# pramasoul/lac

Hardware: AMD Instinct MI355X
Metric: encoded symbols/sec at vocab=32000, batch=4096 streams; bit-exact round-trip (higher is better)
Workload: dtype u32; 1 GPU; c3: vocab=32000, 4096 streams/GPU, 16 symbols/stream per job, prec=48, uint32 pmf rows; vocab=32000, streams=4096, prec=48, pmf_bits=32, input=pmf, parallelism=streams sharded over 1 GPU(s)

## Files before the change

### lac_amd/csrc/lac_encode.hip

```cpp
#include "lac_host.h"
#include "lac_drain.h"
#include "lac_wire.h"

#include <type_traits>

namespace {

#if LAC_ENC_PHASES
__device__ unsigned long long g_enc_phase[8];
#endif

template <typename E, int VEC>
__global__ __launch_bounds__(256) void k_row_stats(const E *__restrict__ pmf, int64_t step_stride,
                                                   int64_t stream_stride, const int32_t *__restrict__ sym,
                                                   int64_t B, int64_t rows, int64_t V, int64_t t0,
                                                   RowStats *__restrict__ out, const EncState *states,
                                                   const int64_t *__restrict__ slen) {
    const int lane = (int)lane_id();
    const int64_t r = (int64_t)blockIdx.x * kWavesPerBlock + (threadIdx.x >> 6);
    if (r >= rows) return;
    const int64_t t = t0 + r / B, b = r % B;
    if (slen && !live_row(slen, b, states[b].nsym, r / B)) return;
    const RowSums rs = row_reduce<E, VEC>(pmf + t * step_stride + b * stream_stride, V, sym[t * B + b]);
    if (lane == 0) {
        RowStats st;
        if (rs.T >> 64) {
            st.lo = st.hi = st.tot = 0;
            st.minp = 1;
        } else {
            st.lo = (uint64_t)rs.lo;
            st.hi = (uint64_t)rs.lo + rs.ps;
            st.tot = (uint64_t)rs.T;
            st.minp = rs.T ? rs.minp : 0;
        }
        st.inv_tot = st.tot ? 1.0 / (double)st.tot : 0.0;
        st.pad = 0;
        out[r] = st;
    }
}

struct SP {
    uint64_t lo, hi, tot, flo, fhi, fthr;
    int n, prec;
    uint64_t cap_words, *pa, *pc;
    int lane;
};
template <bool CEIL, bool T32, bool FT>
__device__ inline int straight_steps(const SP &sp, EncState &st, int64_t &l, int64_t &h, bool &ok) {
    auto store = [&](uint64_t idx, uint64_t wa, uint64_t wc) {
        if (sp.lane == 0) { sp.pa[idx] = wa; sp.pc[idx] = wc; }
    };
    typedef typename std::conditional<T32, uint32_t, uint64_t>::type CT;
    struct Row {
        CT lo, hi, T;
        uint64_t fl, fh, ft;
    };
    auto rd = [&](int j) {
        Row r;
        if constexpr (T32) {
            r.lo = (uint32_t)__builtin_amdgcn_readlane((int)(uint32_t)sp.lo, j);
            r.hi = (uint32_t)__builtin_amdgcn_readlane((int)(uint32_t)sp.hi, j);
            r.T = (uint32_t)__builtin_amdgcn_readlane((int)(uint32_t)sp.tot, j);
        } else {
            r.lo = readlane_u64(sp.lo, j);
            r.hi = readlane_u64(sp.hi, j);
            r.T = readlane_u64(sp.tot, j);
        }
        r.fl = readlane_u64(sp.flo, j);
        r.fh = readlane_u64(sp.fhi, j);
        r.ft = FT ? readlane_u64(sp.fthr, j) : 0;
        return r;
    };
    const int n = sp.n, prec = sp.prec;
    const int64_t nsym0 = st.nsym;
    Row nx = rd(0);
    int i = 0;
    int kk = 0;
    uint64_t e = 0;
    bool fudged = false;
    while (i < n) {
        for (; i < n; i++) {
            const Row r = nx;
            nx = rd(i + 1 < n ? i + 1 : i);
            const uint64_t w = (uint64_t)(h - l + 1);
            if constexpr (FT) {
                if (!nonneg_uni((int64_t)(w - r.ft))) {
                    fudged = true;
                    break;
                }
            }
            uint64_t a, bb;
            if constexpr (T32) {
                a = frac_mul_div32<CEIL>(r.fl, r.lo, w, r.T);
                bb = frac_mul_div32<CEIL>(r.fh, r.hi, w, r.T);
            } else {
                a = frac_mul_div<true>(r.fl, r.lo, w, r.T, CEIL);
                bb = frac_mul_div<true>(r.fh, r.hi, w, r.T, CEIL);
            }
            h = l + (int64_t)bb - 1;
            l = l + (int64_t)a;
            const uint64_t d = (uint64_t)(h - l);
            const int sh = bitlen64(d);
            kk = prec - sh;
            e = kk > 0 ? (uint64_t)l >> sh : 0;
            l = (int64_t)(((uint64_t)l - (e << sh)) << kk);
            h = l + (int64_t)((d + 1) << kk) - 1;
            const int off0 = (int)(st.L & 63);
            const int avail = off0 ? 64 - off0 : 0;
            if (__builtin_expect(kk > avail, 0)) break;
            st.wc |= (e >> kk) << ((64 - off0) & 63);
            st.wa |= (e & ((1ull << kk) - 1)) << ((64 - off0 - kk) & 63);
            st.L += (uint64_t)kk;
        }
        if (i >= n) break;
        if constexpr (FT) {
            if (fudged) break;
        }
        if (!plane_append(st.L, st.wa, st.wc, kk, e, sp.cap_words, store)) {
            st.err = LAC_E_CAPACITY;
            ok = false;
            break;
        }
        i++;
    }
    st.nsym = nsym0 + i;
    return i;
}

template <typename E, int MAP>
__global__ __launch_bounds__(256) void k_encode(const RowStats *__restrict__ stats, const int32_t *__restrict__ sym,
                                                int64_t B, int64_t t0, int64_t nsteps, const E *pmf,
                                                int64_t step_stride, int64_t stream_stride, int64_t V, int prec,
                                                EncState *states, uint64_t *planeA, uint64_t *planeC,
                                                uint64_t cap_words, uint64_t *trace, int mapping,
                                                bool allow_fudge, const int64_t *__restrict__ slen) {
    const int lane = (int)lane_id();
    const int64_t b = (int64_t)blockIdx.x * kWavesPerBlock + wave_in_block();
    if (b >= B) return;
    EncState st = states[b];
    if (slen) {
        nsteps = live_steps(slen, b, st.nsym, nsteps);
        if (nsteps == 0) return;
    }
    if (st.err || st.nflush >= 0) {
        if (lane == 0 && !st.err && st.nflush >= 0) { st.err = LAC_E_STATE; st.err_step = st.nsym; states[b] = st; }
        return;
    }
    uint64_t *pa = planeA + (uint64_t)b * cap_words, *pc = planeC + (uint64_t)b * cap_words;
    int64_t l = (int64_t)rfl_u64((uint64_t)st.l), h = (int64_t)rfl_u64((uint64_t)st.h);
    st.L = rfl_u64(st.L);
    st.wa = rfl_u64(st.wa);
    st.wc = rfl_u64(st.wc);
    st.nsym = (int64_t)rfl_u64((uint64_t)st.nsym);
#if LAC_ENC_PHASES
    PhaseClock clock, *clk = &clock;
    clock.start();
#else
    NoClock *clk = nullptr;
#endif
    bool ok = true;
    for (int64_t g0 = 0; g0 < nsteps && ok; g0 += 64) {
        const int n = (int)((nsteps - g0) < 64 ? (nsteps - g0) : 64);
        RowStats my = {0, 0, 0, 0, 0.0, 0};
        int32_t mys = 0;
        if (lane < n) {
            my = stats[(g0 + lane) * B + b];
            mys = sym[(t0 + g0 + lane) * B + b];
        }
        const bool frac_ok = lane < n && !(my.tot >> 62);
        const uint64_t flo = frac_ok ? row_frac(my.lo, my.tot) : kNoFrac;
        const uint64_t fhi = frac_ok ? row_frac(my.hi, my.tot) : kNoFrac;
        int i0 = 0;
        if constexpr (sizeof(E) == 8) {
            const uint64_t half = 1ull << (prec - 1);
            const bool lfast = lane >= n || (frac_ok && my.tot != 0 && my.hi > my.lo && (uint32_t)mys < (uint32_t)V &&
                                             (MAP != LAC_MAP_FLOOR || ((my.tot - 1) >> (prec - 1)) < my.hi - my.lo));
            const uint64_t d0 = (uint64_t)(h - l);
            if (!trace && prec <= 61 && __ballot(!lfast) == 0 && nonneg_uni((int64_t)(d0 - half)) &&
                !(d0 >> prec)) {
                constexpr bool CEIL = MAP != LAC_MAP_FLOOR;
                const bool t32 = __ballot(lane < n && (my.tot >> 32)) == 0;
                const bool ft = CEIL && __ballot(lane < n && my.tot > half) != 0;
                uint64_t ftl = 0;
                if (ft) {
                    ftl = lane < n && my.minp ? div_floor((u128)my.tot + (my.minp - 1), my.minp) : 0;
                    ftl = ftl < (1ull << 62) ? ftl : (1ull << 62);
                }
                SP sp{my.lo, my.hi, my.tot, flo, fhi, ftl, n, prec, cap_words, pa, pc, lane};
                if (t32)
                    i0 = ft ? straight_steps<CEIL, true, true>(sp, st, l, h, ok)
                            : straight_steps<CEIL, true, false>(sp, st, l, h, ok);
                else
                    i0 = ft ? straight_steps<CEIL, false, true>(sp, st, l, h, ok)
                            : straight_steps<CEIL, false, false>(sp, st, l, h, ok);
                if (!ok || i0 >= n) continue;
            }
        }
        if (i0 == 0) {
            const uint64_t half = 1ull << (prec - 1);
            const bool lfast = lane >= n || (frac_ok && my.tot != 0 && my.tot <= half && !(my.tot >> 32) &&
                                             my.hi > my.lo && (uint32_t)mys < (uint32_t)V);
            const uint64_t d0 = (uint64_t)(h - l);
            if (!trace && prec <= 61 && __ballot(!lfast) == 0 && nonneg_uni((int64_t)(d0 - half)) &&
                !(d0 >> prec)) {
                constexpr bool CEIL = MAP != LAC_MAP_FLOOR;
                const int64_t nsym0 = st.nsym;
                auto store = [&](uint64_t idx, uint64_t wa, uint64_t wc) {
                    if (lane == 0) { pa[idx] = wa; pc[idx] = wc; }
                };
                auto rd = [&](int j, uint32_t &lo, uint32_t &hi, uint32_t &T, uint64_t &fl, uint64_t &fh) {
                    lo = (uint32_t)__builtin_amdgcn_readlane((int)(uint32_t)my.lo, j);
                    hi = (uint32_t)__builtin_amdgcn_readlane((int)(uint32_t)my.hi, j);
                    T = (uint32_t)__builtin_amdgcn_readlane((int)(uint32_t)my.tot, j);
                    fl = readlane_u64(flo, j);
                    fh = readlane_u64(fhi, j);
                };
                uint32_t nlo, nhi, nT;
                uint64_t nfl, nfh;
                rd(0, nlo, nhi, nT, nfl, nfh);
                int i = 0;
                int kk = 0;
                uint64_t e = 0;
                while (i < n) {
                    for (; i < n; i++) {
                        uint32_t lo, hi, T;
                        uint64_t fl, fh;
                        lo = nlo, hi = nhi, T = nT, fl = nfl, fh = nfh;
                        rd(i + 1 < n ? i + 1 : i, nlo, nhi, nT, nfl, nfh);
                        const uint64_t w = (uint64_t)(h - l + 1);
                        const uint64_t a = frac_mul_div32<CEIL>(fl, lo, w, T), bb = frac_mul_div32<CEIL>(fh, hi, w, T);
                        h = l + (int64_t)bb - 1;
                        l = l + (int64_t)a;
                        const uint64_t d = (uint64_t)(h - l);
                        const int sh = bitlen64(d);
                        kk = prec - sh;
                        e = kk > 0 ? (uint64_t)l >> sh : 0;
                        l = (int64_t)(((uint64_t)l - (e << sh)) << kk);
                        h = l + (int64_t)((d + 1) << kk) - 1;
                        const int off0 = (int)(st.L & 63);
                        const int avail = off0 ? 64 - off0 : 0;
                        if (__builtin_expect(kk > avail, 0)) break;
                        st.wc |= (e >> kk) << ((64 - off0) & 63);
                        st.wa |= (e & ((1ull << kk) - 1)) << ((64 - off0 - kk) & 63);
                        st.L += (uint64_t)kk;
                    }
                    if (i >= n) break;
                    if (!plane_append(st.L, st.wa, st.wc, kk, e, cap_words, store)) {
                        st.err = LAC_E_CAPACITY;
                        ok = false;
                        break;
                    }
                    i++;
                }
                st.nsym = nsym0 + i;
                continue;
            }
        }
        uint64_t fthr = lane < n && my.minp ? div_floor((u128)my.tot + (my.minp - 1), my.minp) : 0;
        fthr = fthr < (1ull << 62) ? fthr : (1ull << 62);
        if (clk) clk->mark(4);
        for (int i = i0; i < n; i++) {
            const uint64_t lo = readlane_u64(my.lo, i), hi = readlane_u64(my.hi, i);
            const uint64_t T = readlane_u64(my.tot, i), minp = readlane_u64(my.minp, i);
            const uint64_t invb = readlane_u64(__builtin_bit_cast(uint64_t, my.inv_tot), i);
            const uint64_t fl = readlane_u64(flo, i), fh = readlane_u64(fhi, i), ft = readlane_u64(fthr, i);
            const int64_t s = __builtin_amdgcn_readlane(mys, i);
            const int64_t t = t0 + g0 + i;
            const E *row = pmf + t * step_stride + b * stream_stride;
            if (clk) clk->mark(0);
            if (!coder_step<E, true>(st, l, h, lo, hi, T, minp, s, row, V, prec, pa, pc, cap_words,
                                     trace ? trace + 2 * (t * B + b) : nullptr, lane, MAP,
                                     __builtin_bit_cast(double, invb), allow_fudge, fl, fh, ft, clk)) {
                ok = false;
                break;
            }
        }
    }
    if (lane == 0) store_state(st, l, h, pa, pc, cap_words, &states[b]);
#if LAC_ENC_PHASES
    if (lane == 0) {
        for (int k = 0; k < 5; k++) atomicAdd(&g_enc_phase[k], (unsigned long long)clock.acc[k]);
        atomicAdd(&g_enc_phase[6], (unsigned long long)st.nsym);
    }
#endif
}


template <typename E, int VEC>
__global__ LAC_ENC_BOUNDS void k_encode_fused(const E *__restrict__ pmf, int64_t step_stride,
                                                      int64_t stream_stride, const int32_t *__restrict__ sym,
                                                      int64_t B, int64_t t0, int64_t nsteps, int64_t V, int prec,
                                                      EncState *states, uint64_t *planeA, uint64_t *planeC,
                                                      uint64_t cap_words, uint64_t *trace, uint64_t *nbits, int flags,
                                                      int mapping, int term, const int64_t *__restrict__ slen) {
    const int lane = (int)lane_id();
    const int64_t b = (int64_t)blockIdx.x * kStreamWaves + (threadIdx.x >> 6);
    if (b >= B) return;
    EncState st = (flags & kReset) ? fresh_state(prec) : states[b];
    uint64_t *pa = planeA + (uint64_t)b * cap_words, *pc = planeC + (uint64_t)b * cap_words;
    if (slen) nsteps = live_steps(slen, b, st.nsym, nsteps);
    if (st.err || st.nflush >= 0) {
        if (!st.err && st.nflush >= 0 && nsteps > 0) { st.err = LAC_E_STATE; st.err_step = st.nsym; }
        if (lane == 0) {
            states[b] = st;
            if (flags & kFinish) nbits[b] = st.err ? 0 : st.L;
        }
        return;
    }
    int64_t l = st.l, h = st.h;
    RowGroup<E, VEC> buf;
    for (int64_t i = 0; i < nsteps; i++) {
        const int64_t t = t0 + i;
        const E *row = pmf + t * step_stride + b * stream_stride;
        row_group_load<E, VEC>(buf, row, 0, V / VEC);
        const int64_t s = sym[t * B + b];
        const RowSums rs = row_reduce_pf<E, VEC>(row, V, s, buf);
        if (rs.T >> 64) { st.err = (s < 0 || s >= V) ? LAC_E_SYMBOL_RANGE : LAC_E_TABLE; break; }
        const uint64_t lo = (uint64_t)rs.lo;
        if (!coder_step<E>(st, l, h, lo, lo + rs.ps, (uint64_t)rs.T, rs.minp, s, row, V, prec, pa, pc, cap_words,
                           trace ? trace + 2 * (t * B + b) : nullptr, lane, mapping))
            break;
    }
    if (lane == 0) {
        store_state(st, l, h, pa, pc, cap_words, &st);
        if (flags & kFinish) finish_stream(st, pa, pc, cap_words, prec, &nbits[b], term);
        states[b] = st;
    }
}

__global__ __launch_bounds__(256) void k_finish(EncState *states, uint64_t *planeA, uint64_t *planeC,
                                                uint64_t cap_words, int64_t B, int prec, uint64_t *nbits, int term) {
    const int64_t b = (int64_t)blockIdx.x * blockDim.x + threadIdx.x;
    if (b >= B) return;
    EncState st = states[b];
    finish_stream(st, planeA + (uint64_t)b * cap_words, planeC + (uint64_t)b * cap_words, cap_words, prec, &nbits[b],
                  term);
    states[b] = st;
}

__device__ inline uint64_t block_excl_sum1024(uint64_t v, uint64_t *wsum, uint64_t &total) {
    const int w = threadIdx.x >> 6;
    const uint64_t inc = wave_incl_scan_u64(v);
    if ((threadIdx.x & 63) == 63) wsum[w] = inc;
    __syncthreads();
    uint64_t before = 0;
    total = 0;
    for (int i = 0; i < 16; i++) {
        const uint64_t x = wsum[i];
        before += i < w ? x : 0;
        total += x;
    }
    __syncthreads();
    return before + inc - v;
}

__global__ __launch_bounds__(1024) void k_pack(const uint64_t *__restrict__ planes, uint64_t pstride,
                                               uint64_t cap_words, const uint64_t *__restrict__ nbits_all,
                                               int64_t B, int hdr, uint8_t *__restrict__ dst, uint64_t dst_bytes,
                                               const uint64_t *__restrict__ base_in, uint64_t *__restrict__ ends,
                                               uint64_t *__restrict__ lens) {
    __shared__ uint64_t wsum[16];
// ... 155 lines not shown
}

__global__ __launch_bounds__(64 * kWavesPerBlock) void k_enc_drain(EncState *states, uint64_t *planeA,
                                                                   uint64_t *planeC, uint64_t cap_words, int64_t B,
                                                                   int prec, uint8_t *dst, uint64_t dst_stride,
                                                                   uint64_t *fill) {
    const int lane = (int)lane_id();
    const int64_t b = (int64_t)blockIdx.x * kWavesPerBlock + wave_in_block();
    if (b >= B) return;
    const EncState st = states[b];
    if (drain::is_idle(__builtin_amdgcn_readfirstlane(st.err), __builtin_amdgcn_readfirstlane(st.nflush),
                       rfl_u64(st.L)))
        return;
    const uint64_t L = rfl_u64(st.L), wlast = (L - 1) >> 6;
    if (wlast >= cap_words) return;
    const uint64_t wa = rfl_u64(st.wa), wc = rfl_u64(st.wc);
    uint64_t *pa = planeA + (uint64_t)b * cap_words, *pc = planeC + (uint64_t)b * cap_words;
    uint64_t g = 0, sg = 0, cy = 0;
    const bool certain = drain::is_certain((int64_t)rfl_u64((uint64_t)st.l), (int64_t)rfl_u64((uint64_t)st.h), prec);
    if (certain) {
        g = wlast;
        sg = drain::resolve_word(wa, wc, 0, &cy);
    } else {
        for (uint64_t top = wlast; top > 0; top = top > 64 ? top - 64 : 0) {
            const bool in = (uint64_t)lane < top;
            const uint64_t i = in ? top - 1 - (uint64_t)lane : 0;
            const uint64_t a = pa[i], c = pc[i];
            uint64_t co;
            const uint64_t s = drain::resolve_word(a, c, 0, &co);
            const uint64_t m = __ballot(in && drain::is_guard(a, c));
            if (m) {
                const int first = __builtin_ctzll(m);
                g = top - 1 - (uint64_t)first;
                sg = rfl_u64(shfl_u64(s, first));
                cy = (__ballot(co != 0) >> first) & 1;
                break;
            }
        }
    }
    if (g == 0) return;
    const uint64_t f = rfl_u64(fill[b]);
    if (!drain::slot_fits(g, f, dst_stride)) return;
    uint64_t *out = reinterpret_cast<uint64_t *>(dst + (uint64_t)b * dst_stride + f);
    uint64_t carry = cy;
    for (uint64_t top = g; top > 0; top = top > 64 ? top - 64 : 0) {
        const bool in = (uint64_t)lane < top;
        const uint64_t i = in ? top - 1 - (uint64_t)lane : 0;
        const uint64_t a0 = pa[i], c0 = pc[i];
        const uint64_t a = in ? a0 : 0, c = in ? c0 : 0;
        uint64_t co;
        const uint64_t s = drain::resolve_word(a, c, 0, &co);
        const uint64_t gen = __ballot(co != 0), prop = __ballot(s == ~0ull);
        uint64_t cout;
        const uint64_t cin = drain::block_carries(gen, prop, carry, &cout);
        if (in) out[i] = drain::to_big_endian(s + ((cin >> lane) & 1));
        carry = cout;
    }
    const uint64_t nk = wlast - g + 1;
    for (uint64_t base = 0; base < nk; base += 64) {
        const uint64_t j = base + (uint64_t)lane;
        const bool in = j < nk;
        const uint64_t src = g + (in ? j : 0);
        uint64_t a = pa[src], c = pc[src];
        if (j == 0) { a = sg; c = 0; }
        if (j == nk - 1) { a = certain ? sg : wa; c = certain ? 0 : wc; }
        if (in) { pa[j] = a; pc[j] = c; }
    }
    if (lane == 0) {
        states[b].L = L - 64 * g;
        if (certain) { states[b].wa = sg; states[b].wc = 0; }
        fill[b] = f + 8 * g;
    }
}

__global__ void k_enc_reset(EncState *states, int64_t B, int prec) {
    const int64_t b = (int64_t)blockIdx.x * blockDim.x + threadIdx.x;
    if (b >= B) return;
    states[b] = fresh_state(prec);
}

}


template <typename E, int VEC>
static int encode_impl(lac_ctx *c, const E *pmf, int64_t step_stride, int64_t stream_stride, const int32_t *sym,
                       int64_t steps, uint64_t *trace, hipStream_t st, int flags) {
    const unsigned blocks = (unsigned)((c->B + kWavesPerBlock - 1) / kWavesPerBlock);
    const bool fused = c->path == LAC_PATH_FUSED || (c->path == LAC_PATH_AUTO && c->B >= c->fused_min_streams);
    if (fused) {
        ProfScope ps(c, KID_FUSED, st);
        k_encode_fused<E, VEC><<<(unsigned)((c->B + kStreamWaves - 1) / kStreamWaves), 64 * kStreamWaves, 0, st>>>(
            pmf, step_stride, stream_stride, sym, c->B, 0, steps, c->V, c->prec, c->enc, c->planeA, c->planeC,
            c->cap_words, trace, c->nbits, flags, c->mapping, c->term, stream_lengths(c));
        CHECK_LAUNCH();
        return LAC_OK;
    }
    if (flags & kReset) {
        k_enc_reset<<<(unsigned)((c->B + 255) / 256), 256, 0, st>>>(c->enc, c->B, c->prec);
        CHECK_LAUNCH();
    }
    for (int64_t t0 = 0; t0 < steps; t0 += c->chunk_steps) {
        const int64_t n = (steps - t0) < c->chunk_steps ? (steps - t0) : c->chunk_steps;
        const int64_t rows = n * c->B;
        {
            ProfScope ps(c, KID_ROW_STATS, st);
            k_row_stats<E, VEC><<<(unsigned)((rows + kWavesPerBlock - 1) / kWavesPerBlock), 64 * kWavesPerBlock, 0,
                                  st>>>(pmf, step_stride, stream_stride, sym, c->B, rows, c->V, t0, c->stats, c->enc,
                                        stream_lengths(c));
        }
        CHECK_LAUNCH();
        {
            ProfScope ps(c, KID_ENCODE, st);
            if (c->mapping == LAC_MAP_FLOOR)
                k_encode<E, LAC_MAP_FLOOR><<<blocks, 64 * kWavesPerBlock, 0, st>>>(
                    c->stats, sym, c->B, t0, n, pmf, step_stride, stream_stride, c->V, c->prec, c->enc, c->planeA,
                    c->planeC, c->cap_words, trace, c->mapping, true, stream_lengths(c));
            else
                k_encode<E, LAC_MAP_CEIL><<<blocks, 64 * kWavesPerBlock, 0, st>>>(
                    c->stats, sym, c->B, t0, n, pmf, step_stride, stream_stride, c->V, c->prec, c->enc, c->planeA,
                    c->planeC, c->cap_words, trace, c->mapping, true, stream_lengths(c));
        }
        CHECK_LAUNCH();
    }
    if (flags & kFinish) {
        ProfScope ps(c, KID_FINISH, st);
        k_finish<<<(unsigned)((c->B + 255) / 256), 256, 0, st>>>(c->enc, c->planeA, c->planeC, c->cap_words, c->B,
                                                                 c->prec, c->nbits, c->term);
        CHECK_LAUNCH();
    }
    return LAC_OK;
}

static int encode_dispatch(lac_ctx *c, const void *pmf_dev, int64_t step_stride, int64_t stream_stride,
                           const int32_t *sym_dev, int64_t steps, uint64_t *trace_dev, void *stream, int flags) {
    if (!c || (steps > 0 && (!pmf_dev || !sym_dev))) return fail(LAC_E_ARG, "NULL argument");
    if (steps < 0 || step_stride < 0 || stream_stride < 0) return fail(LAC_E_ARG, "negative size/stride");
    if (steps == 0 && !flags) return LAC_OK;
    HIPCHK(hipSetDevice(c->device));
    c->mode = 0;
    hipStream_t st = S(stream);
    const uintptr_t p = (uintptr_t)pmf_dev;
    if (c->pmf_bits == 32) {
        const bool vec = (p % 16 == 0) && c->V % 4 == 0 && step_stride % 4 == 0 && stream_stride % 4 == 0;
        return vec ? encode_impl<uint32_t, 4>(c, (const uint32_t *)pmf_dev, step_stride, stream_stride, sym_dev, steps,
                                              trace_dev, st, flags)
                   : encode_impl<uint32_t, 1>(c, (const uint32_t *)pmf_dev, step_stride, stream_stride, sym_dev, steps,
                                              trace_dev, st, flags);
    }
    const bool vec = (p % 16 == 0) && c->V % 2 == 0 && step_stride % 2 == 0 && stream_stride % 2 == 0;
    return vec ? encode_impl<uint64_t, 2>(c, (const uint64_t *)pmf_dev, step_stride, stream_stride, sym_dev, steps,
                                          trace_dev, st, flags)
               : encode_impl<uint64_t, 1>(c, (const uint64_t *)pmf_dev, step_stride, stream_stride, sym_dev, steps,
                                          trace_dev, st, flags);
}


int enc_reset_launch(lac_ctx *c, hipStream_t st) {
    k_enc_reset<<<(unsigned)((c->B + 255) / 256), 256, 0, st>>>(c->enc, c->B, c->prec);
    CHECK_LAUNCH();
    return LAC_OK;
}

int enc_stats_launch(lac_ctx *c, const int32_t *sym, int64_t t0, int64_t n, uint64_t *trace, hipStream_t st) {
    const unsigned blocks = (unsigned)((c->B + kWavesPerBlock - 1) / kWavesPerBlock);
    {
        ProfScope ps(c, KID_ENCODE, st);
        k_encode<uint32_t, LAC_MAP_CEIL><<<blocks, 64 * kWavesPerBlock, 0, st>>>(
            c->stats, sym, c->B, t0, n, (const uint32_t *)nullptr, 0, 0, c->V, c->prec, c->enc, c->planeA,
            c->planeC, c->cap_words, trace, LAC_MAP_CEIL, false, stream_lengths(c));
    }
    CHECK_LAUNCH();
    return LAC_OK;
}

int enc_finish_launch(lac_ctx *c, int term, hipStream_t st) {
    ProfScope ps(c, KID_FINISH, st);
    k_finish<<<(unsigned)((c->B + 255) / 256), 256, 0, st>>>(c->enc, c->planeA, c->planeC, c->cap_words, c->B,
                                                             c->prec, c->nbits, term);
    CHECK_LAUNCH();
    return LAC_OK;
}

extern "C" {

#if LAC_ENC_PHASES
int lac_debug_enc_phases(uint64_t *out8, int reset) {
    HIPCHK(hipDeviceSynchronize());
    HIPCHK(hipMemcpyFromSymbol(out8, HIP_SYMBOL(g_enc_phase), sizeof(uint64_t) * 8));
    if (reset) {
        const unsigned long long z[8] = {0, 0, 0, 0, 0, 0, 0, 0};
        HIPCHK(hipMemcpyToSymbol(HIP_SYMBOL(g_enc_phase), z, sizeof z));
    }
    return LAC_OK;
}
#endif

int lac_encode_reset(lac_ctx *c, void *stream) {
    if (!c) return fail(LAC_E_ARG, "ctx is NULL");
    HIPCHK(hipSetDevice(c->device));
    c->mode = 0;
    c->finished = 0;
    c->open = 0;
    c->fsm_busy = 0;
    k_enc_reset<<<(unsigned)((c->B + 255) / 256), 256, 0, S(stream)>>>(c->enc, c->B, c->prec);
    CHECK_LAUNCH();
    return LAC_OK;
}

int lac_encode_rebase(lac_ctx *c, void *stream) {
    if (!c) return fail(LAC_E_ARG, "ctx is NULL");
    if (c->mode != 0) return fail(LAC_E_STATE, "context is decoding");
    HIPCHK(hipSetDevice(c->device));
    k_enc_rebase<<<(unsigned)((c->B + 255) / 256), 256, 0, S(stream)>>>(c->enc, c->B);
    CHECK_LAUNCH();
    return LAC_OK;
}

int lac_encode_drain(lac_ctx *c, uint8_t *dst_dev, uint64_t dst_stride_bytes, uint64_t *fill_dev, void *stream) {
    if (!c) return fail(LAC_E_ARG, "ctx is NULL");
    if (c->mode != 0) return fail(LAC_E_STATE, "context is decoding");
    if (c->finished)
        return fail(LAC_E_STATE, "the streams are finished (plane A holds their packed bytes): lac_encode_reset first");
    if (!dst_dev || !fill_dev) return fail(LAC_E_ARG, "dst_dev and fill_dev must not be NULL");
    if ((uintptr_t)dst_dev % 8 || (uintptr_t)fill_dev % 8 || dst_stride_bytes % 8)
        return fail(LAC_E_ARG, "dst_dev, fill_dev and dst_stride_bytes must be multiples of 8");
    HIPCHK(hipSetDevice(c->device));
    k_enc_drain<<<(unsigned)((c->B + kWavesPerBlock - 1) / kWavesPerBlock), 64 * kWavesPerBlock, 0, S(stream)>>>(
        c->enc, c->planeA, c->planeC, c->cap_words, c->B, c->prec, dst_dev, dst_stride_bytes, fill_dev);
    CHECK_LAUNCH();
    return LAC_OK;
}

int lac_encode(lac_ctx *c, const void *pmf_dev, int64_t step_stride, int64_t stream_stride, const int32_t *sym_dev,
               int64_t steps, uint64_t *trace_dev, void *stream) {
    if (c && c->mode != 0) return fail(LAC_E_STATE, "context is decoding; call lac_encode_reset first");
    const int rc = encode_dispatch(c, pmf_dev, step_stride, stream_stride, sym_dev, steps, trace_dev, stream, 0);
    if (rc == LAC_OK && steps > 0) enc_mark_open(c);
    return rc;
}

int lac_encode_job(lac_ctx *c, const void *pmf_dev, int64_t step_stride, int64_t stream_stride,
                   const int32_t *sym_dev, int64_t steps, uint64_t *trace_dev, void *stream) {
    const int rc = encode_dispatch(c, pmf_dev, step_stride, stream_stride, sym_dev, steps, trace_dev, stream,
                                   kReset | kFinish);
    if (rc == LAC_OK) enc_mark_finished(c);
    return rc;
}

int lac_encode_finish(lac_ctx *c, void *stream) {
    if (!c) return fail(LAC_E_ARG, "ctx is NULL");
    if (c->mode != 0) return fail(LAC_E_STATE, "context is decoding");
    HIPCHK(hipSetDevice(c->device));
    ProfScope ps(c, KID_FINISH, S(stream));
    enc_mark_finished(c);
    k_finish<<<(unsigned)((c->B + 255) / 256), 256, 0, S(stream)>>>(c->enc, c->planeA, c->planeC, c->cap_words, c->B,
// ... 147 lines not shown
```

### lac_amd/csrc/lac_host.h

```cpp
#pragma once
#include <stdarg.h>
#include <stddef.h>
#include <string>
#include <vector>

#include "lac_dev.h"
#include "lac_select.h"
#include "lac_fsm.h"
#include "lac_count.h"
#include "lac_history.h"

struct lac_ctx {
    int device = 0, prec = 0, pmf_bits = 32;
    int64_t V = 0, B = 0;
    uint64_t cap_bits = 0, cap_words = 0;
    RowStats *stats = nullptr;
    EncState *enc = nullptr;
    DecState *dec = nullptr;
    TailState *tail = nullptr;
    uint64_t *planeA = nullptr, *planeC = nullptr, *nbits = nullptr;
    uint64_t *own_planeA = nullptr, *own_nbits = nullptr;
    const uint8_t *dbits = nullptr;
    uint64_t dstride = 0;
    const uint64_t *dnbits = nullptr;
// ... 41 lines not shown
    bool has_len = false;
    void *fsm = nullptr;
    FsmLayout fsm_y = {};
    bool fsm_has_next = false;
    int32_t *fsm_state = nullptr;
    int *fsm_flag = nullptr;
    int fsm_busy = 0;
    uint32_t *cnt = nullptr;
    int32_t *cnt_past = nullptr;
    void *cnt_row = nullptr;
    CountLayout cnt_y = {};
    uint32_t cnt_w[4] = {0, 0, 0, 0};
    const uint64_t *hist_L = nullptr;
    int32_t *hist_ring = nullptr;
    int32_t *hist_pasti = nullptr;
    int32_t *hist_M = nullptr;
    void *hist_row = nullptr;
    int *hist_flag = nullptr;
    int hist_P = 0;
    bool prof = false;
    std::vector<hipEvent_t> ev_pool;
    std::vector<std::pair<int, std::pair<hipEvent_t, hipEvent_t>>> ev_used;
    size_t ev_next = 0;
};

enum { KID_ROW_STATS = 0, KID_ENCODE = 1, KID_FINISH = 2, KID_DECODE = 3, KID_FUSED = 4, KID_DECODE_WAVE = 5,
       KID_Q1_STATS = 6, KID_Q1_DECODE = 7, KID_COUNT = 8 };

static inline hipEvent_t ev_get(lac_ctx *c) {
    if (c->ev_next == c->ev_pool.size()) {
        hipEvent_t e;
        if (hipEventCreate(&e) != hipSuccess) return nullptr;
        c->ev_pool.push_back(e);
    }
    return c->ev_pool[c->ev_next++];
}

struct ProfScope {
    lac_ctx *c;
    int kid;
    hipStream_t st;
    hipEvent_t a = nullptr, b = nullptr;
    ProfScope(lac_ctx *c_, int kid_, hipStream_t st_) : c(c_), kid(kid_), st(st_) {
        if (c->prof && kid >= 0) {
            a = ev_get(c);
            b = ev_get(c);
            if (a && b) (void)hipEventRecord(a, st);
        }
    }
    ~ProfScope() {
        if (c->prof && a && b) {
            (void)hipEventRecord(b, st);
            c->ev_used.push_back({kid, {a, b}});
        }
    }
};

int fail(int code, const char *fmt, ...) __attribute__((format(printf, 2, 3)));

#define HIPCHK(x)                                                                          \
    do {                                                                                   \
        hipError_t e_ = (x);                                                               \
        if (e_ != hipSuccess) return fail(LAC_E_HIP, "%s: %s", #x, hipGetErrorString(e_)); \
    } while (0)

#define CHECK_LAUNCH() HIPCHK(hipGetLastError())

static inline hipStream_t S(void *s) { return reinterpret_cast<hipStream_t>(s); }

static inline const int64_t *stream_lengths(const lac_ctx *c) { return c->has_len ? c->slen : nullptr; }

static inline void enc_mark_open(lac_ctx *c) {
    c->open = 1;
    c->finished = 0;
}
static inline void enc_mark_finished(lac_ctx *c) {
    c->open = 0;
    c->finished = 1;
    c->fin_planeA = c->planeA;
    c->fin_nbits = c->nbits;
}

int enc_reset_launch(lac_ctx *c, hipStream_t st);
int enc_stats_launch(lac_ctx *c, const int32_t *sym, int64_t t0, int64_t n, uint64_t *trace, hipStream_t st);
int enc_finish_launch(lac_ctx *c, int term, hipStream_t st);
int ensure_chunk_buffers(lac_ctx *c);
```

### lac_amd/csrc/lac_logits.hip

```cpp
#include "lac_host.h"
#include "lac_dec_dev.h"

namespace {

__constant__ uint32_t c_q1_tab[LAC_Q1_TAB_SIZE] = LAC_Q1_TAB_INIT;


#ifndef LAC_Q1_DEFER_DEC
#define LAC_Q1_DEFER_DEC 0
#endif

typedef uint32_t u32x4 __attribute__((ext_vector_type(4)));
typedef short s16x2 __attribute__((ext_vector_type(2)));
__device__ inline s16x2 as_s16x2(uint32_t w) {
    s16x2 r;
    __builtin_memcpy(&r, &w, 4);
    return r;
}

template <typename LT> struct LogitN { static constexpr int N = 16 / sizeof(LT); };

template <typename LT>
__device__ inline float logit_at(const u32x4 &v, int j) {
    if constexpr (sizeof(LT) == 2) {
// ... 1665 lines not shown
        const int64_t need = (a.rows + NR - 1) / NR, cap = (int64_t)c->cus * per_cu;
        const unsigned grid = (unsigned)(need < cap ? need : cap);
        ProfScope ps(c, gate ? -1 : KID_Q1_STATS, st);
        k_q1_stats<LT, RW, R, DEC, MULTI, PF, NWB><<<grid, 64 * NWB, 0, st>>>(LAC_Q1_ARGS, gate);
        CHECK_LAUNCH();
        return LAC_OK;
    }
}

static int q1_group_setup(lac_ctx *c, const Q1Args &a, hipStream_t st, const Q1Group &g, bool dec, unsigned *grid,
                          int *rpx_out) {
    if (!c->pxch) HIPCHK(hipMalloc(&c->pxch, sizeof(uint64_t) * (8 * (int64_t)c->cus + 1)));
    const int64_t spx = (int64_t)(c->cus / 8) * g.nrb, rcap = spx / g.k, rneed = (a.rows + 7) / 8;
    const int64_t rpx = rneed < rcap ? rneed : rcap;
    *grid = (unsigned)(8 * ((rpx * g.k + g.nrb - 1) / g.nrb));
    *rpx_out = (int)rpx;
    HIPCHK(hipMemsetAsync(c->pxch, 0, sizeof(uint64_t) * (2 * g.nrb * (int64_t)*grid + 1), st));
    if (dec) HIPCHK(hipMemsetAsync(c->q1chunks, 0, sizeof(uint64_t) * 64 * a.rows, st));
    else HIPCHK(hipMemsetAsync(c->stats, 0, sizeof(RowStats) * a.rows, st));
    return LAC_OK;
}

template <typename LT, bool DEC>
static int q1_group_repair(lac_ctx *c, const Q1Args &a, hipStream_t st, const Q1Plan &p, unsigned grid) {
    c->xch_abort = 2 * p.group.nrb * (int64_t)grid;
    return q1_tiled_launch<LT, DEC>(c, a, st, p, c->pxch + c->xch_abort);
}

template <typename LT, bool DEC, bool GROUP>
static int q1_slot_launch(lac_ctx *c, const Q1Args &a, hipStream_t st, const Q1Plan &p) {
    const bool wide = p.family == Q1_WIDE || p.family == Q1_WIDE_GROUP;
    const int64_t nrb = wide ? 1 : 1024 / p.nt, need = (a.rows + nrb - 1) / nrb;
    unsigned grid = (unsigned)(need < c->cus ? need : c->cus);
    int rpx = 0, rc;
    if (GROUP && (rc = q1_group_setup(c, a, st, p.group, DEC, &grid, &rpx))) return rc;
#define LAC_Q1_SLOT_ARGS LAC_Q1_ARGS, GROUP ? c->pxch : nullptr, GROUP ? p.group.split : 0, GROUP ? p.group.k : 1, rpx
#define LAC_Q1_RL(REP, LASTN, NT)                       \
    if (p.rep == REP && p.lastn == LASTN && p.nt == NT) \
    k_q1_stats_rl<LT, DEC, REP, LASTN, NT, GROUP><<<grid, 1024, 0, st>>>(LAC_Q1_SLOT_ARGS)
    {
        ProfScope ps(c, KID_Q1_STATS, st);
        if (wide && (GROUP || !p.wide_slots)) {
            k_q1_stats_wide<LT, kQ1WideR, DEC, GROUP><<<grid, 512, 0, st>>>(LAC_Q1_SLOT_ARGS);
        } else if (wide) {
            if constexpr (!GROUP)
                k_q1_stats_wide<LT, kQ1WideR, DEC, false, kQ1WideL><<<grid, 512, 0, st>>>(LAC_Q1_SLOT_ARGS);
        } else LAC_Q1_RL(16, kRLLastTrim, 1024);
        else LAC_Q1_RL(kRLRep, 1024, 1024);
        else LAC_Q1_RL(16, 320, 512);
        else LAC_Q1_RL(kRLRep, 512, 512);
        else LAC_Q1_RL(kRLRep, 256, 256);
        else if constexpr (!DEC) {
            LAC_Q1_RL(16, 192, 256);
        } else if constexpr (!GROUP) {
            LAC_Q1_RL(kRLRep, 192, 256);
        }
        CHECK_LAUNCH();
    }
#undef LAC_Q1_RL
#undef LAC_Q1_SLOT_ARGS
    if constexpr (GROUP) return q1_group_repair<LT, DEC>(c, a, st, p, grid);
    return LAC_OK;
}

template <typename LT, bool DEC>
static int q1_launch(lac_ctx *c, const Q1Args &a, hipStream_t st, const Q1Plan &p) {
    if (p.family == Q1_TILED) return q1_tiled_launch<LT, DEC>(c, a, st, p);
    if (p.family == Q1_RL || p.family == Q1_WIDE) return q1_slot_launch<LT, DEC, false>(c, a, st, p);
    return q1_slot_launch<LT, DEC, true>(c, a, st, p);
}

template <typename LT, bool DEC>
static int q1_stats(lac_ctx *c, const Q1Args &a, hipStream_t st) {
    Q1Plan p;
    if (q1_plan(c->cus, c->V, (int)sizeof(LT), DEC, c->q1_shape, &p))
        return fail(LAC_E_ARG, "q1 shape %d does not hold a row of %lld vectors", c->q1_shape,
                    (long long)(c->V / LogitN<LT>::N));
    return q1_launch<LT, DEC>(c, a, st, p);
}

template <typename LT>
static int q1_encode(lac_ctx *c, const Q1Args &a0, int64_t steps, uint64_t *trace, hipStream_t st, int flags) {
    int rc;
    if ((flags & kReset) && (rc = enc_reset_launch(c, st))) return rc;
    for (int64_t t0 = 0; t0 < steps; t0 += c->chunk_steps) {
        const int64_t n = (steps - t0) < c->chunk_steps ? (steps - t0) : c->chunk_steps;
        Q1Args a = a0;
        a.rows = n * c->B;
        a.t0 = t0;
        if ((rc = q1_stats<LT, false>(c, a, st))) return rc;
        if ((rc = enc_stats_launch(c, a.sym, t0, n, trace, st))) return rc;
    }
    if ((flags & kFinish) && (rc = enc_finish_launch(c, LAC_TERM_FLUSH, st))) return rc;
    return LAC_OK;
}

template <typename LT>
static int q1_decode(lac_ctx *c, const Q1Args &a0, int64_t steps, int32_t *out, hipStream_t st) {
    int rc0 = ensure_chunk_buffers(c);
    if (rc0) return rc0;
    const unsigned blocks = (unsigned)((c->B + kWavesPerBlock - 1) / kWavesPerBlock);
    const int64_t nvec = c->V / LogitN<LT>::N;
    for (int64_t t0 = 0; t0 < steps; t0 += c->chunk_steps) {
        const int64_t n = (steps - t0) < c->chunk_steps ? (steps - t0) : c->chunk_steps;
        Q1Args a = a0;
        a.rows = n * c->B;
        a.t0 = t0;
        int rc = q1_stats<LT, true>(c, a, st);
        if (rc) return rc;
        ProfScope ps(c, KID_Q1_DECODE, st);
        const int64_t G = q1_groups_per_chunk(nvec);
#define LAC_Q1_DEC(GC)                                                                                            \
    k_q1_decode<LT, GC><<<blocks, 64 * kWavesPerBlock, 0, st>>>((const LT *)a.lg, a.ss, a.bs, t0, n, c->V, c->prec, \
                                                               a.xsh, G, c->q1chunks, c->q1m, c->dec, c->dbits,    \
                                                               c->dstride, c->dnbits, out, c->B, stream_lengths(c))
        if (c->prec > 50)
            k_q1_decode<LT, 0, false><<<blocks, 64 * kWavesPerBlock, 0, st>>>(
                (const LT *)a.lg, a.ss, a.bs, t0, n, c->V, c->prec, a.xsh, G, c->q1chunks, c->q1m, c->dec, c->dbits,
                c->dstride, c->dnbits, out, c->B, stream_lengths(c));
        else switch (G) {
        case 1: LAC_Q1_DEC(1); break;
        case 2: LAC_Q1_DEC(2); break;
        case 3: LAC_Q1_DEC(3); break;
        case 4: LAC_Q1_DEC(4); break;
        case 5: LAC_Q1_DEC(5); break;
        case 6: LAC_Q1_DEC(6); break;
        case 7: LAC_Q1_DEC(7); break;
        case 8: LAC_Q1_DEC(8); break;
        default: LAC_Q1_DEC(0); break;
        }
#undef LAC_Q1_DEC
        CHECK_LAUNCH();
    }
    return LAC_OK;
}

template <typename LT>
static int q1_step_decode(lac_ctx *c, const Q1Args &a, const Q1StepPlan &p, int32_t *out, hipStream_t st) {
    ProfScope ps(c, KID_Q1_DECODE, st);
#define LAC_Q1_STEP_DEC(R, SMALL)                                                                               \
    k_q1_step_dec<LT, R, SMALL><<<(unsigned)c->B, p.threads, 0, st>>>((const LT *)a.lg, a.bs, c->V, c->prec, a.xsh, \
                                                                      c->dec, c->dbits, c->dstride, c->dnbits, out, \
                                                                      stream_lengths(c))
    if (c->prec > 50) {
        if (p.R == 4) LAC_Q1_STEP_DEC(4, false);
        else if (p.R == 8) LAC_Q1_STEP_DEC(8, false);
        else LAC_Q1_STEP_DEC(16, false);
    } else {
        if (p.R == 4) LAC_Q1_STEP_DEC(4, true);
        else if (p.R == 8) LAC_Q1_STEP_DEC(8, true);
        else LAC_Q1_STEP_DEC(16, true);
    }
#undef LAC_Q1_STEP_DEC
    CHECK_LAUNCH();
    return LAC_OK;
}

template <typename LT>
static int q1_step_encode(lac_ctx *c, const Q1Args &a, const Q1StepPlan &p, uint64_t *trace, hipStream_t st) {
    ProfScope ps(c, KID_ENCODE, st);
#define LAC_Q1_STEP_ENC(R)                                                                                        \
    k_q1_step_enc<LT, R><<<(unsigned)c->B, p.threads, 0, st>>>((const LT *)a.lg, a.bs, a.sym, c->V, c->prec, a.xsh, \
                                                               c->enc, c->planeA, c->planeC, c->cap_words, trace,   \
                                                               stream_lengths(c))
    if (p.R == 4) LAC_Q1_STEP_ENC(4);
    else if (p.R == 8) LAC_Q1_STEP_ENC(8);
    else LAC_Q1_STEP_ENC(16);
#undef LAC_Q1_STEP_ENC
    CHECK_LAUNCH();
    return LAC_OK;
}

static int q1_step_choose(lac_ctx *c, int logit_type, Q1StepPlan *p) {
    *p = q1_step_plan(c->cus, c->V, logit_type == LAC_LOGITS_BF16 ? 2 : 4, c->B, c->q1_step);
    if (p->rc)
        return fail(p->rc, "the fused logits step holds rows of <= %d vectors for <= %lld streams", kQ1StepMaxVec,
// ... 130 lines not shown
```

Baseline: 54.05 million symbols/s.

## Fold stream reset and finish into the encode kernel via job template flag

Adds a JOB template parameter to k_encode so the first chunk initialises the stream state in registers and the last chunk runs the flush/finish inside the same kernel. This drops the separate k_enc_reset and k_finish launches on the non-fused and Q1 encode paths. The finish step is rewritten as a wave-wide carry-propagating pass over the plane words instead of a single-thread loop. The cost is more template instantiations and added register pressure in the encode kernel. If the auto path picks the fused kernel for this batch size, none of this code runs.

Result: slower. 53.02 million symbols/s (-1.9%).

```diff
diff --git a/lac_amd/csrc/lac_encode.hip b/lac_amd/csrc/lac_encode.hip
--- a/lac_amd/csrc/lac_encode.hip
+++ b/lac_amd/csrc/lac_encode.hip
@@ -20,7 +20,7 @@
     const int64_t r = (int64_t)blockIdx.x * kWavesPerBlock + (threadIdx.x >> 6);
     if (r >= rows) return;
     const int64_t t = t0 + r / B, b = r % B;
-    if (slen && !live_row(slen, b, states[b].nsym, r / B)) return;
+    if (slen && !live_row(slen, b, states ? states[b].nsym : 0, r / B)) return;
     const RowSums rs = row_reduce<E, VEC>(pmf + t * step_stride + b * stream_stride, V, sym[t * B + b]);
     if (lane == 0) {
         RowStats st;
@@ -127,23 +127,106 @@
     return i;
 }
 
-template <typename E, int MAP>
+template <int JOB>
+__device__ inline void job_idle(EncState &st, uint64_t *pa, uint64_t *pc, uint64_t cap_words, int prec,
+                                uint64_t *nbits_slot, int term, EncState *slot) {
+    if constexpr ((JOB & kFinish) != 0) finish_stream(st, pa, pc, cap_words, prec, nbits_slot, term);
+    *slot = st;
+}
+
+__device__ inline void finish_stream_wave(EncState &st, uint64_t *pa, uint64_t *pc, uint64_t cap_words, int prec,
+                                          uint64_t *nbits_slot, int term, int lane, EncState *slot) {
+    int8_t fd[8];
+    const bool common = !st.err && st.nflush < 0 && term != LAC_TERM_ACSAMPLER;
+    const int m = common ? flush_digits(st.l, st.h, prec, fd) : -1;
+    const uint64_t L = st.L, Lf = L + (uint64_t)(m > 0 ? m : 0), nwords = (Lf + 63) >> 6;
+    if (m < 0 || nwords > cap_words) {
+        if (lane == 0) {
+            finish_stream(st, pa, pc, cap_words, prec, nbits_slot, term);
+            *slot = st;
+        }
+        return;
+    }
+    int64_t F = 0;
+    for (int i = 0; i < m; i++) F = F * 2 + fd[i];
+    const int pad = (int)(nwords * 64 - Lf);
+    i128 carry = (i128)F * ((i128)1 << pad);
+    const int64_t last = L ? (int64_t)((L - 1) >> 6) : -1;
+    __builtin_amdgcn_fence(__ATOMIC_SEQ_CST, "wavefront");
+    for (int64_t top = (int64_t)nwords; top > 0; top -= 64) {
+        const int64_t i = top - 1 - lane;
+        uint64_t a = 0, c = 0;
+        if (i == last) {
+            a = st.wa;
+            c = st.wc;
+        } else if (i >= 0 && i < last) {
+            a = pa[i];
+            c = pc[i];
+        }
+        const int n = (int)(top < 64 ? top : 64);
+        uint64_t out = 0;
+        for (int j = 0; j < n; j++) {
+            const i128 sm = (i128)(u128)readlane_u64(a, j) + (i128)(u128)readlane_u64(c, j) + carry;
+            if (lane == j) out = bswap64((uint64_t)sm);
+            carry = sm >> 64;
+        }
+        if (i >= 0) pa[i] = out;
+    }
+    if (carry != 0) st.err = LAC_E_ARG;
+    st.nflush = m;
+    for (int i = 0; i < 8; i++) st.flush[i] = i < m ? fd[i] : 0;
+    st.L = Lf;
+    if (lane == 0) {
+        *nbits_slot = st.err ? 0 : Lf;
+        *slot = st;
+    }
+}
+
+template <typename E, int MAP, int JOB = 0>
 __global__ __launch_bounds__(256) void k_encode(const RowStats *__restrict__ stats, const int32_t *__restrict__ sym,
                                                 int64_t B, int64_t t0, int64_t nsteps, const E *pmf,
                                                 int64_t step_stride, int64_t stream_stride, int64_t V, int prec,
                                                 EncState *states, uint64_t *planeA, uint64_t *planeC,
                                                 uint64_t cap_words, uint64_t *trace, int mapping,
-                                                bool allow_fudge, const int64_t *__restrict__ slen) {
+                                                bool allow_fudge, const int64_t *__restrict__ slen,
+                                                uint64_t *nbits, int term) {
     const int lane = (int)lane_id();
     const int64_t b = (int64_t)blockIdx.x * kWavesPerBlock + wave_in_block();
     if (b >= B) return;
-    EncState st = states[b];
+    EncState st;
+    if constexpr ((JOB & kReset) != 0) {
+        st.l = 0;
+        st.h = ((int64_t)1 << prec) - 1;
+        st.L = st.wa = st.wc = 0;
+        st.nsym = 0;
+        st.err = 0;
+        st.nflush = -1;
+        st.err_step = -1;
+        for (int i = 0; i < 8; i++) st.flush[i] = 0;
+    } else {
+        st = states[b];
+    }
     if (slen) {
         nsteps = live_steps(slen, b, st.nsym, nsteps);
-        if (nsteps == 0) return;
+        if (nsteps == 0) {
+            if constexpr (JOB != 0) {
+                if (lane == 0)
+                    job_idle<JOB>(st, planeA + (uint64_t)b * cap_words, planeC + (uint64_t)b * cap_words, cap_words,
+                                  prec, &nbits[b], term, &states[b]);
+            }
+            return;
+        }
     }
     if (st.err || st.nflush >= 0) {
-        if (lane == 0 && !st.err && st.nflush >= 0) { st.err = LAC_E_STATE; st.err_step = st.nsym; states[b] = st; }
+        if constexpr (JOB != 0) {
+            if (lane == 0) {
+                if (!st.err && st.nflush >= 0) { st.err = LAC_E_STATE; st.err_step = st.nsym; }
+                job_idle<JOB>(st, planeA + (uint64_t)b * cap_words, planeC + (uint64_t)b * cap_words, cap_words, prec,
+                              &nbits[b], term, &states[b]);
+            }
+        } else {
+            if (lane == 0 && !st.err && st.nflush >= 0) { st.err = LAC_E_STATE; st.err_step = st.nsym; states[b] = st; }
+        }
         return;
     }
     uint64_t *pa = planeA + (uint64_t)b * cap_words, *pc = planeC + (uint64_t)b * cap_words;
@@ -276,7 +359,13 @@
             }
         }
     }
-    if (lane == 0) store_state(st, l, h, pa, pc, cap_words, &states[b]);
+    if constexpr ((JOB & kFinish) != 0) {
+        EncState fin;
+        store_state(st, l, h, pa, pc, cap_words, &fin);
+        finish_stream_wave(fin, pa, pc, cap_words, prec, &nbits[b], term, lane, &states[b]);
+    } else {
+        if (lane == 0) store_state(st, l, h, pa, pc, cap_words, &states[b]);
+    }
 #if LAC_ENC_PHASES
     if (lane == 0) {
         for (int k = 0; k < 5; k++) atomicAdd(&g_enc_phase[k], (unsigned long long)clock.acc[k]);
@@ -598,6 +687,27 @@
 }
 
 
+template <typename E, int MAP>
+static int encode_launch(lac_ctx *c, int job, const int32_t *sym, int64_t t0, int64_t n, const E *pmf,
+                         int64_t step_stride, int64_t stream_stride, uint64_t *trace, int mapping, bool allow_fudge,
+                         int term, hipStream_t st) {
+    const unsigned blocks = (unsigned)((c->B + kWavesPerBlock - 1) / kWavesPerBlock);
+#define LAC_ENC(JOB)                                                                                               \
+    k_encode<E, MAP, JOB><<<blocks, 64 * kWavesPerBlock, 0, st>>>(                                                 \
+        c->stats, sym, c->B, t0, n, pmf, step_stride, stream_stride, c->V, c->prec, c->enc, c->planeA, c->planeC, \
+        c->cap_words, trace, mapping, allow_fudge, stream_lengths(c), c->nbits, term)
+    {
+        ProfScope ps(c, KID_ENCODE, st);
+        if (job == 0) LAC_ENC(0);
+        else if (job == kReset) LAC_ENC(kReset);
+        else if (job == kFinish) LAC_ENC(kFinish);
+        else LAC_ENC(kReset | kFinish);
+    }
+#undef LAC_ENC
+    CHECK_LAUNCH();
+    return LAC_OK;
+}
+
 template <typename E, int VEC>
 static int encode_impl(lac_ctx *c, const E *pmf, int64_t step_stride, int64_t stream_stride, const int32_t *sym,
                        int64_t steps, uint64_t *trace, hipStream_t st, int flags) {
@@ -611,38 +721,23 @@
         CHECK_LAUNCH();
         return LAC_OK;
     }
-    if (flags & kReset) {
-        k_enc_reset<<<(unsigned)((c->B + 255) / 256), 256, 0, st>>>(c->enc, c->B, c->prec);
-        CHECK_LAUNCH();
-    }
-    for (int64_t t0 = 0; t0 < steps; t0 += c->chunk_steps) {
+    for (int64_t t0 = 0; t0 < steps || (t0 == 0 && flags); t0 += c->chunk_steps) {
         const int64_t n = (steps - t0) < c->chunk_steps ? (steps - t0) : c->chunk_steps;
         const int64_t rows = n * c->B;
-        {
+        const int job = (t0 == 0 ? flags & kReset : 0) | (t0 + n >= steps ? flags & kFinish : 0);
+        if (rows > 0) {
             ProfScope ps(c, KID_ROW_STATS, st);
             k_row_stats<E, VEC><<<(unsigned)((rows + kWavesPerBlock - 1) / kWavesPerBlock), 64 * kWavesPerBlock, 0,
-                                  st>>>(pmf, step_stride, stream_stride, sym, c->B, rows, c->V, t0, c->stats, c->enc,
-                                        stream_lengths(c));
+                                  st>>>(pmf, step_stride, stream_stride, sym, c->B, rows, c->V, t0, c->stats,
+                                        (job & kReset) ? nullptr : c->enc, stream_lengths(c));
         }
         CHECK_LAUNCH();
-        {
-            ProfScope ps(c, KID_ENCODE, st);
-            if (c->mapping == LAC_MAP_FLOOR)
-                k_encode<E, LAC_MAP_FLOOR><<<blocks, 64 * kWavesPerBlock, 0, st>>>(
-                    c->stats, sym, c->B, t0, n, pmf, step_stride, stream_stride, c->V, c->prec, c->enc, c->planeA,
-                    c->planeC, c->cap_words, trace, c->mapping, true, stream_lengths(c));
-            else
-                k_encode<E, LAC_MAP_CEIL><<<blocks, 64 * kWavesPerBlock, 0, st>>>(
-                    c->stats, sym, c->B, t0, n, pmf, step_stride, stream_stride, c->V, c->prec, c->enc, c->planeA,
-                    c->planeC, c->cap_words, trace, c->mapping, true, stream_lengths(c));
-        }
-        CHECK_LAUNCH();
-    }
-    if (flags & kFinish) {
-        ProfScope ps(c, KID_FINISH, st);
-        k_finish<<<(unsigned)((c->B + 255) / 256), 256, 0, st>>>(c->enc, c->planeA, c->planeC, c->cap_words, c->B,
-                                                                 c->prec, c->nbits, c->term);
-        CHECK_LAUNCH();
+        const int rc = c->mapping == LAC_MAP_FLOOR
+                           ? encode_launch<E, LAC_MAP_FLOOR>(c, job, sym, t0, n, pmf, step_stride, stream_stride, trace,
+                                                             c->mapping, true, c->term, st)
+                           : encode_launch<E, LAC_MAP_CEIL>(c, job, sym, t0, n, pmf, step_stride, stream_stride, trace,
+                                                            c->mapping, true, c->term, st);
+        if (rc) return rc;
     }
     return LAC_OK;
 }
@@ -677,16 +772,10 @@
     return LAC_OK;
 }
 
-int enc_stats_launch(lac_ctx *c, const int32_t *sym, int64_t t0, int64_t n, uint64_t *trace, hipStream_t st) {
-    const unsigned blocks = (unsigned)((c->B + kWavesPerBlock - 1) / kWavesPerBlock);
-    {
-        ProfScope ps(c, KID_ENCODE, st);
-        k_encode<uint32_t, LAC_MAP_CEIL><<<blocks, 64 * kWavesPerBlock, 0, st>>>(
-            c->stats, sym, c->B, t0, n, (const uint32_t *)nullptr, 0, 0, c->V, c->prec, c->enc, c->planeA,
-            c->planeC, c->cap_words, trace, LAC_MAP_CEIL, false, stream_lengths(c));
-    }
-    CHECK_LAUNCH();
-    return LAC_OK;
+int enc_stats_launch(lac_ctx *c, const int32_t *sym, int64_t t0, int64_t n, uint64_t *trace, int job, int term,
+                     hipStream_t st) {
+    return encode_launch<uint32_t, LAC_MAP_CEIL>(c, job, sym, t0, n, (const uint32_t *)nullptr, 0, 0, trace,
+                                                 LAC_MAP_CEIL, false, term, st);
 }
 
 int enc_finish_launch(lac_ctx *c, int term, hipStream_t st) {
diff --git a/lac_amd/csrc/lac_host.h b/lac_amd/csrc/lac_host.h
--- a/lac_amd/csrc/lac_host.h
+++ b/lac_amd/csrc/lac_host.h
@@ -147,6 +147,7 @@
 }
 
 int enc_reset_launch(lac_ctx *c, hipStream_t st);
-int enc_stats_launch(lac_ctx *c, const int32_t *sym, int64_t t0, int64_t n, uint64_t *trace, hipStream_t st);
+int enc_stats_launch(lac_ctx *c, const int32_t *sym, int64_t t0, int64_t n, uint64_t *trace, int job, int term,
+                     hipStream_t st);
 int enc_finish_launch(lac_ctx *c, int term, hipStream_t st);
 int ensure_chunk_buffers(lac_ctx *c);
diff --git a/lac_amd/csrc/lac_logits.hip b/lac_amd/csrc/lac_logits.hip
--- a/lac_amd/csrc/lac_logits.hip
+++ b/lac_amd/csrc/lac_logits.hip
@@ -1771,16 +1771,15 @@
 template <typename LT>
 static int q1_encode(lac_ctx *c, const Q1Args &a0, int64_t steps, uint64_t *trace, hipStream_t st, int flags) {
     int rc;
-    if ((flags & kReset) && (rc = enc_reset_launch(c, st))) return rc;
-    for (int64_t t0 = 0; t0 < steps; t0 += c->chunk_steps) {
+    for (int64_t t0 = 0; t0 < steps || (t0 == 0 && flags); t0 += c->chunk_steps) {
         const int64_t n = (steps - t0) < c->chunk_steps ? (steps - t0) : c->chunk_steps;
+        const int job = (t0 == 0 ? flags & kReset : 0) | (t0 + n >= steps ? flags & kFinish : 0);
         Q1Args a = a0;
         a.rows = n * c->B;
         a.t0 = t0;
-        if ((rc = q1_stats<LT, false>(c, a, st))) return rc;
-        if ((rc = enc_stats_launch(c, a.sym, t0, n, trace, st))) return rc;
-    }
-    if ((flags & kFinish) && (rc = enc_finish_launch(c, LAC_TERM_FLUSH, st))) return rc;
+        if (a.rows > 0 && (rc = q1_stats<LT, false>(c, a, st))) return rc;
+        if ((rc = enc_stats_launch(c, a.sym, t0, n, trace, job, LAC_TERM_FLUSH, st))) return rc;
+    }
     return LAC_OK;
 }
 
```
